# gabrielspmoreira/chameleon_recsys

Measured on AMD Instinct MI355X. Metric: NAR training sessions/sec, higher is better.
Workload: dtype f32

## Files before the change

chameleon_recsys_amd/_lib.py:

```python
import ctypes
import os
from ctypes import c_double, c_float, c_int, c_int32, c_int64, c_long, c_size_t, c_uint32, c_void_p

_HERE = os.path.dirname(os.path.abspath(__file__))
LIB_PATH = os.path.join(_HERE, "libchameleon_nar.so")

P = c_void_p

_SIGNATURES = {
    "cham_neg_sample_workspace_bytes": (c_size_t, [c_int, c_int, c_int]),
    "cham_neg_sample": (c_int, [P, c_int, c_int, P, c_int, c_uint32, c_uint32, c_int, c_int, c_int, c_int, P, P, P, P, P,
                                P, c_size_t, P]),
    "cham_ctx_assemble": (c_int, [P, P, c_int, P, c_int, P, P, P, P, P, P]),
    "cham_set_log_bases": (c_int, [c_float, c_float]),
    "cham_step_ints": (c_int, [P, P, P, P, c_int64, c_int, c_int, P, c_int, P, P, P, P, P, P]),
    "cham_item_dynamic_raw": (c_int, [P, P, c_int, P, P, P, P, P]),
    "cham_norm_stats_from_recent": (c_int, [P, c_int, c_int64, P, P, P, P, P]),
    "cham_norm_stats_from_buffer": (c_int, [P, c_int, c_int64, P, P, P, P, P]),
    "cham_norm_stats_from_rows": (c_int, [P, P, P, c_int, P, P]),
    "cham_row_weights": (c_int, [P, c_int, P, c_size_t, c_int, P, P, P, P]),
    "cham_item_assemble": (c_int, [P, c_int, c_int, c_int, P, c_int, P, c_int, P, P, P, P, c_int, P, P, P, P, P, P]),
    "cham_item_assemble_lds": (c_int, [P, c_int, c_int, c_int, P, c_int, P, c_int, P, P, P, P, c_int, P, c_int, P, c_int, P, P, P, P, P, P]),
    "cham_feature_bwd": (c_int, [P, P, c_int, c_int, P, P, P]),
    "cham_feature_bwd_workspace_bytes": (c_size_t, [c_int]),
# ... 30 lines not shown
    "cham_split2h": (c_int, [P, c_int, c_int, c_int, P, c_int64, c_int, P, c_int64, c_int, P, c_int, P]),
    "cham_gemm_h2": (c_int, [P, c_int64, c_int, P, P, c_int64, c_int, P, c_int, P, c_int, c_int, c_int, c_int, P, c_int, P, c_int, c_int, c_int,
                             P, c_size_t, c_int, P]),
    "cham_h2b_block_elements": (c_int, []),
    "cham_gemm_h2b": (c_int, [P, c_int64, c_int, P, P, c_int64, c_int, P, c_int, P, c_int, c_int, c_int, c_int, P, c_int, P, c_int, c_int, c_int,
                              P, c_size_t, c_int, c_int, c_int, c_int, P]),
    "cham_combine_fwd_h2b": (c_int, [P, P, c_int, c_int, c_int, c_int, P, P, c_int64, P, c_int, P]),
    "cham_dm_mulpred_h2_blk": (c_int, [P, c_int, c_int, P, c_int64, P, P, P, P, c_int, c_int, c_int, P, c_int64, P, P, P, P]),
    "cham_gemm_h2_launch_counts": (None, [P, c_int]),
    "cham_gemm_h2_set_nt_wide": (c_int, [c_int]),
    "cham_combine_fwd_h2": (c_int, [P, P, c_int, c_int, c_int, c_int, P, P, c_int64, P, P]),
    "cham_mulpred_bwd_h2": (c_int, [P, P, P, c_int, c_int, c_int, P, P, c_int64, P, P, P]),
    "cham_dm_mulpred_h2": (c_int, [P, c_int, c_int, P, c_int64, P, P, c_int, c_int, c_int, P, c_int64, P, P, P, P]),
    "cham_dm_mulpred_h2h": (c_int, [P, c_int, c_int, P, c_int64, P, P, P, P, c_int, c_int, c_int, P, c_int64, P, P, P, P]),
    "cham_dm_mulpred_b16": (c_int, [P, c_int, c_int, P, P, P, c_int, c_int, c_int, P, P, P, P]),
    "cham_gemm_b16": (c_int, [P, c_int, c_int, P, c_int, c_int, P, c_int, c_int, c_int, c_int, c_int, P, c_int, P, c_int, c_int, c_int,
                              P, c_size_t, c_int, P]),
    "cham_gemm_b16_set_variant": (None, [c_int]),
    "cham_gemm_b16_launch_counts": (None, [P, c_int]),
    "cham_gemm_set_variant": (None, [c_int]),
    "cham_gemm_launch_counts": (None, [P, c_int]),
    "cham_combine_fwd": (c_int, [P, P, c_int, c_int, c_int, c_int, P, P, c_long, c_long, P]),
    "cham_combine_bwd_workspace_bytes": (c_size_t, [c_int, c_int, c_int, c_int]),
    "cham_combine_bwd": (c_int, [P, c_int, c_int, c_int, c_int, P, P, P, P, c_size_t, P]),
    "cham_combine_bwd_gs": (c_int, [P, c_int, c_int, c_int, c_int, P, P, P, P, c_size_t, P, c_size_t, P]),
    "cham_gemm_h2_groupsum_bytes": (c_size_t, [c_int, c_int, c_int]),
    "cham_gemm_h2_dgrad_gs": (c_int, [P, c_int64, c_int, P, P, c_int64, c_int, P, P, c_int, c_int, c_int, c_int, P, c_int, c_int, c_int, c_int, P,
                                      c_size_t, P]),
    "cham_combine_fwd_b16": (c_int, [P, P, c_int, c_int, c_int, c_int, P, P, P]),
    "cham_combine_bwd_b16": (c_int, [P, P, c_int, c_int, c_int, c_int, P, P, P, P, c_size_t, P]),
# ... 62 lines not shown
def load():
    global _lib
    if _lib is not None:
        return _lib
    if not os.path.exists(LIB_PATH):
        raise ChameleonLibError(
            "HIP extension %s is missing - run `python -c 'import __graft_entry__ as g; g.build()'` "
            "(hipcc --offload-arch=gfx950).  There is no CPU fallback." % LIB_PATH)
    lib = ctypes.CDLL(LIB_PATH)
    for name, (res, args) in _SIGNATURES.items():
        fn = getattr(lib, name)
        fn.restype = res
        fn.argtypes = args
    lib.cham_gemm_h2_set_nt_wide(1 if os.environ.get("CHAM_H2_NT_WIDE", "1") == "1" else 0)
    lib.cham_gemm_b16_dma_set_nt_wide(1 if os.environ.get("CHAM_B16_NT_WIDE", "1") == "1" else 0)
    _lib = lib
    return lib


def check(rc, what):
    if rc != 0:
        raise ChameleonLibError("%s failed with code %d" % (what, rc))


def ptr(t):
    return None if t is None else t.data_ptr()
```

chameleon_recsys_amd/csrc/dm_fused.hip:

```cpp
#include "gemm_shared.h"
#include <type_traits>

#define DMF_NT 2
#define DMF_COLS (32 * DMF_NT)
#define DMF_PLANE (DMF_COLS * 128)
#define DMF_HALF (3 * DMF_PLANE)
#define DMF_RED_OFF (2 * DMF_HALF)
#define DMF_RED_BYTES (8 * 4 * DMF_COLS * 4)

static_assert(DMF_NT == 2, "the epilogue packs exactly two tiles' columns per lane");

struct DmfParams {
    const float* dS1; int lds1;
    const __bf16* W; long long w_ps;
    const float* Z2c; const float* pred;
    __bf16* out; long long out_ps;
    const H2Scale* osc;
    const H2Scale* sa; const H2Scale* sw;
    float* dpred; float* b2part;
    int C, BT, NC, PW;
    int out_blocked;
};

__device__ __forceinline__ void dmf_dma_one(unsigned lds, unsigned voff, const u32x4& r) {
    unsigned keep;
    asm volatile(
        "s_nop 4\n\t"
        "s_mov_b32 %0, m0\n\t"
        "s_mov_b32 m0, %1\n\ts_nop 0\n\tbuffer_load_dwordx4 %2, %3, 0 offen lds\n\t"
        "s_mov_b32 m0, %0"
        : "=&s"(keep) : "s"(lds), "v"(voff), "s"(r) : "memory");
}

template <int MODE>
__global__ __launch_bounds__(512) void k_dm_mulpred_fused(DmfParams p) {
    constexpr bool H2 = MODE == 1 || MODE == 3, B16 = MODE == 2, F16P = MODE == 3;
    constexpr int NPL = B16 ? 1 : (F16P ? 2 : 3);
    extern __shared__ __attribute__((aligned(1024))) unsigned char dmf_smem[];
    const int lane = threadIdx.x & 63, wave = __builtin_amdgcn_readfirstlane(threadIdx.x >> 6);
    const int l31 = lane & 31, hh = lane >> 5;
    const int NC = p.NC, C = p.C;
    const int pos0 = blockIdx.x * p.PW;
    const int npos = min(p.PW, p.BT - pos0);
    const int rows_valid = npos * NC;
    const size_t row0 = (size_t)pos0 * NC;
    const int wr0 = 32 * wave;

    bf16x8 AH[8], AM[(B16 || F16P) ? 1 : 8], AL[B16 ? 1 : 8];
    float ginv_a = 1.f, ginv_w = 1.f;
    if constexpr (B16) {
// ... 20 lines not shown
                                __uint_as_float(x[2 * s + 1].w)};
            if constexpr (F16P) {
                const float sa = p.sa->scale;
#pragma unroll
                for (int e = 0; e < 8; ++e) {
                    _Float16 a, c;
                    split2h(v[e] * sa, a, c);
                    AH[s][e] = __builtin_bit_cast(__bf16, a); AL[s][e] = __builtin_bit_cast(__bf16, c);
                }
            } else {
#pragma unroll
                for (int e = 0; e < 8; ++e) { __bf16 a, b, c; split3(v[e], a, b, c); AH[s][e] = a; AM[s][e] = b; AL[s][e] = c; }
            }
        }
    }
    const __amdgpu_buffer_rsrc_t zw = B16 ?
        __builtin_amdgcn_make_buffer_rsrc(const_cast<__bf16*>(reinterpret_cast<const __bf16*>(p.Z2c) + row0 * (size_t)C), 0,
                                          (unsigned)((size_t)rows_valid * C * 2), 0x00020000) :
        __builtin_amdgcn_make_buffer_rsrc(const_cast<float*>(p.Z2c + row0 * (size_t)C), 0, (unsigned)((size_t)rows_valid * C * 4), 0x00020000);
    __amdgpu_buffer_rsrc_t ow[3];
#pragma unroll
    for (int q = 0; q < 3; ++q)
        ow[q] = __builtin_amdgcn_make_buffer_rsrc(p.out + ((H2 && q == 2) || B16 ? 0 : q) * p.out_ps + row0 * (size_t)C, 0, (unsigned)((size_t)rows_valid * C * 2), 0x00020000);
    const bool oblk = H2 && p.out_blocked != 0;
    const unsigned rin = (unsigned)(row0 & 255), tile_bytes = ((unsigned)C >> 5) * (unsigned)(H2B_BLOCK * 2);
    if (oblk) {
#pragma unroll
        for (int q = 0; q < 2; ++q)
            ow[q] = __builtin_amdgcn_make_buffer_rsrc(p.out + q * p.out_ps + (row0 >> 8) * (size_t)((unsigned)C >> 5) * H2B_BLOCK, 0, 2u * tile_bytes, 0x00020000);
    }
    float osc = 1.f;
    if constexpr (H2) osc = p.osc->scale;
    if constexpr (F16P) { ginv_a = p.sa->inv; ginv_w = p.sw->inv; }

// ... 6 lines not shown
        rw[q].x = (unsigned)a; rw[q].y = (unsigned)(a >> 32) & 0xFFFFu; rw[q].z = (unsigned)((size_t)C * 128 * 2); rw[q].w = 0x00020000u;
    }
    unsigned voff;
    {
        const int slot = 8 * wave + (lane >> 3);
        const int piece = (lane & 7) ^ ((slot >> 1) & 7);
        const int col = DMF_NT * (slot & 31) + (slot >> 5);
        voff = (unsigned)(col * 128 + piece * 8) * 2u;
    }
    auto dma_half = [&](int h) {
        const unsigned base = lds_base + (unsigned)(h & 1) * DMF_HALF + (unsigned)wave * 1024u;
        const unsigned add = (unsigned)(((h >> 1) * DMF_COLS) * 128 + (h & 1) * 64) * 2u;
#pragma unroll
        for (int q = 0; q < NPL; ++q) dmf_dma_one(base + (unsigned)q * DMF_PLANE, voff + add, rw[q]);
    };
    unsigned fo[4];
#pragma unroll
    for (int t = 0; t < 4; ++t) fo[t] = (unsigned)(l31 * 128 + (((2 * t + hh) ^ ((l31 >> 1) & 7)) * 16));

    const int pa = wr0 / NC;
    const int bnd = (pa + 1) * NC - wr0;
    const int ntiles = C / DMF_COLS, nhalf = 2 * ntiles;

    dma_half(0);
    dma_half(1);
    floatx16 acc[DMF_NT];
#pragma unroll
    for (int j = 0; j < DMF_NT; ++j)
#pragma unroll
        for (int e = 0; e < 16; ++e) acc[j][e] = 0.f;
    if constexpr (B16) asm volatile("s_waitcnt vmcnt(1)" ::: "memory");
    else if constexpr (F16P) asm volatile("s_waitcnt vmcnt(2)" ::: "memory");
    else asm volatile("s_waitcnt vmcnt(3)" ::: "memory");
    __builtin_amdgcn_fence(__ATOMIC_RELEASE, "workgroup", "local");
    __builtin_amdgcn_s_barrier();
    __builtin_amdgcn_fence(__ATOMIC_ACQUIRE, "workgroup", "local");

    auto mfma_half = [&](auto PARC) {
        constexpr int PAR = decltype(PARC)::value, s0 = PAR * 4;
        const unsigned char* S = dmf_smem + PAR * DMF_HALF;
        __builtin_amdgcn_sched_barrier(0);
#pragma unroll
        for (int t = 0; t < 4; ++t) {
            bf16x8 bh[DMF_NT], bm[DMF_NT], bl[DMF_NT];
#pragma unroll
            for (int j = 0; j < DMF_NT; ++j) {
                bh[j] = *reinterpret_cast<const bf16x8*>(S + fo[t] + j * 4096);
                if constexpr (F16P) {
// ... 21 lines not shown
#pragma unroll
                for (int j = 0; j < DMF_NT; ++j) acc[j] = __builtin_amdgcn_mfma_f32_32x32x16_bf16(AL[s0 + t], bh[j], acc[j], 0, 0, 0);
#pragma unroll
                for (int j = 0; j < DMF_NT; ++j) acc[j] = __builtin_amdgcn_mfma_f32_32x32x16_bf16(AH[s0 + t], bl[j], acc[j], 0, 0, 0);
#pragma unroll
                for (int j = 0; j < DMF_NT; ++j) acc[j] = __builtin_amdgcn_mfma_f32_32x32x16_bf16(AM[s0 + t], bm[j], acc[j], 0, 0, 0);
#pragma unroll
                for (int j = 0; j < DMF_NT; ++j) acc[j] = __builtin_amdgcn_mfma_f32_32x32x16_bf16(AM[s0 + t], bh[j], acc[j], 0, 0, 0);
#pragma unroll
                for (int j = 0; j < DMF_NT; ++j) acc[j] = __builtin_amdgcn_mfma_f32_32x32x16_bf16(AH[s0 + t], bm[j], acc[j], 0, 0, 0);
#pragma unroll
                for (int j = 0; j < DMF_NT; ++j) acc[j] = __builtin_amdgcn_mfma_f32_32x32x16_bf16(AH[s0 + t], bh[j], acc[j], 0, 0, 0);
            }
        }
    };
    for (int h = 0; h < nhalf; ++h) {
        if (h & 1) mfma_half(std::integral_constant<int, 1>{});
        else mfma_half(std::integral_constant<int, 0>{});
        __builtin_amdgcn_sched_barrier(0);
        asm volatile("s_waitcnt vmcnt(0)" ::: "memory");
        if (h & 1) {
            const int col = (h >> 1) * DMF_COLS + DMF_NT * l31;
            float2 pra = make_float2(0.f, 0.f), prb = pra;
            if (pa < npos) pra = *reinterpret_cast<const float2*>(p.pred + (size_t)(pos0 + pa) * C + col);
            if (pa + 1 < npos) prb = *reinterpret_cast<const float2*>(p.pred + (size_t)(pos0 + pa + 1) * C + col);
            float2 sa = make_float2(0.f, 0.f), sb = sa, ca = sa, cb = sa;
            typedef unsigned int u32x2_t __attribute__((ext_vector_type(2)));
            u32x2_t zz[16];
#pragma unroll
            for (int e = 0; e < 16; ++e) {
                const unsigned r = (unsigned)(wr0 + (e & 3) + 8 * (e >> 2) + 4 * hh);
                if constexpr (B16) {
                    const unsigned u = __builtin_amdgcn_raw_buffer_load_b32(zw, (r * (unsigned)C + (unsigned)col) * 2u, 0, 0);
                    zz[e].x = u << 16; zz[e].y = u & 0xFFFF0000u;
                } else {
                    zz[e] = __builtin_amdgcn_raw_buffer_load_b64(zw, (r * (unsigned)C + (unsigned)col) * 4u, 0, 0);
                }
            }
#pragma unroll
            for (int e = 0; e < 16; ++e) {
                const int rr = (e & 3) + 8 * (e >> 2) + 4 * hh;
                const unsigned r = (unsigned)(wr0 + rr);
                const float2 z = make_float2(__uint_as_float(zz[e].x), __uint_as_float(zz[e].y));
                const bool second = rr >= bnd;
                const float2 pr = second ? prb : pra;
                float2 g = make_float2(acc[0][e], acc[1][e]);
                if constexpr (F16P) { g.x = (g.x * ginv_a) * ginv_w; g.y = (g.y * ginv_a) * ginv_w; }
                if constexpr (B16) { g.x = (float)(__bf16)g.x; g.y = (float)(__bf16)g.y; }
                float2 o;
                o.x = g.x * pr.x * (1.f - z.x * z.x); o.y = g.y * pr.y * (1.f - z.y * z.y);
                if constexpr (B16) {
                    typedef __bf16 bf16x2_t __attribute__((ext_vector_type(2)));
                    bf16x2_t ph; ph[0] = (__bf16)o.x; ph[1] = (__bf16)o.y;
                    __builtin_amdgcn_raw_buffer_store_b32(__builtin_bit_cast(unsigned, ph), ow[0], (r * (unsigned)C + (unsigned)col) * 2u, 0, 0);
                    o.x = (float)ph[0]; o.y = (float)ph[1];
                } else if constexpr (H2) {
                    _Float16 h0, l0, h1, l1;
                    split2h(o.x * osc, h0, l0); split2h(o.y * osc, h1, l1);
                    const unsigned ph = (unsigned)h2_keep_sign(h0, o.x) | ((unsigned)h2_keep_sign(h1, o.y) << 16);
                    const unsigned pl = (unsigned)__builtin_bit_cast(unsigned short, l0) | ((unsigned)__builtin_bit_cast(unsigned short, l1) << 16);
                    unsigned oo = (r * (unsigned)C + (unsigned)col) * 2u;
                    if (oblk) {
                        const unsigned lr = rin + r;
                        oo = (int)r < rows_valid ? (lr >> 8) * tile_bytes + ((unsigned)col >> 5) * (unsigned)(H2B_BLOCK * 2) + (lr & 255u) * 64u + ((unsigned)col & 31u) * 2u
                                                 : 0x80000000u;
                    }
                    __builtin_amdgcn_raw_buffer_store_b32(ph, ow[0], oo, 0, 0);
                    __builtin_amdgcn_raw_buffer_store_b32(pl, ow[1], oo, 0, 0);
                } else {
                    typedef __bf16 bf16x2_t __attribute__((ext_vector_type(2)));
                    bf16x2_t ph, pm, pl;
                    __bf16 a, b, c;
                    split3(o.x, a, b, c); ph[0] = a; pm[0] = b; pl[0] = c;
                    split3(o.y, a, b, c); ph[1] = a; pm[1] = b; pl[1] = c;
                    const unsigned oo = (r * (unsigned)C + (unsigned)col) * 2u;
                    __builtin_amdgcn_raw_buffer_store_b32(__builtin_bit_cast(unsigned, ph), ow[0], oo, 0, 0);
                    __builtin_amdgcn_raw_buffer_store_b32(__builtin_bit_cast(unsigned, pm), ow[1], oo, 0, 0);
                    __builtin_amdgcn_raw_buffer_store_b32(__builtin_bit_cast(unsigned, pl), ow[2], oo, 0, 0);
                }
                const float2 gz = make_float2(g.x * z.x, g.y * z.y);
                sb.x += second ? gz.x : 0.f; sb.y += second ? gz.y : 0.f; cb.x += second ? o.x : 0.f; cb.y += second ? o.y : 0.f;
                sa.x += second ? 0.f : gz.x; sa.y += second ? 0.f : gz.y; ca.x += second ? 0.f : o.x; ca.y += second ? 0.f : o.y;
                acc[0][e] = 0.f; acc[1][e] = 0.f;
            }
            float* red = reinterpret_cast<float*>(dmf_smem + DMF_RED_OFF) + (size_t)wave * (4 * DMF_COLS);
            float2 q[4] = {sa, ca, sb, cb};
#pragma unroll
            for (int i = 0; i < 4; ++i) {
                float2 o;
                o.x = __shfl_xor(q[i].x, 32, 64); o.y = __shfl_xor(q[i].y, 32, 64);
                if (hh == 0) *reinterpret_cast<float2*>(red + i * DMF_COLS + DMF_NT * l31) = make_float2(q[i].x + o.x, q[i].y + o.y);
            }
        }
        __builtin_amdgcn_fence(__ATOMIC_RELEASE, "workgroup", "local");
        __builtin_amdgcn_s_waitcnt(0xc07f);
        __builtin_amdgcn_s_barrier();
        __builtin_amdgcn_fence(__ATOMIC_ACQUIRE, "workgroup", "local");
        if (h & 1) {
            const float* redw = reinterpret_cast<const float*>(dmf_smem + DMF_RED_OFF);
            for (int idx = threadIdx.x; idx < npos * DMF_COLS; idx += 512) {
                const int pl = idx / DMF_COLS, c = idx % DMF_COLS;
                float s = 0.f, cs = 0.f;
                const int w_lo = (pl * NC) >> 5, w_hi = min(7, ((pl + 1) * NC - 1) >> 5);
                for (int w = w_lo; w <= w_hi; ++w) {
                    const int slot = (pl == (32 * w) / NC) ? 0 : 1;
                    s += redw[(size_t)w * (4 * DMF_COLS) + slot * (2 * DMF_COLS) + c];
                    cs += redw[(size_t)w * (4 * DMF_COLS) + slot * (2 * DMF_COLS) + DMF_COLS + c];
                }
                const int colg = (h >> 1) * DMF_COLS + c;
                const float pr = p.pred[(size_t)(pos0 + pl) * C + colg];
                p.dpred[(size_t)(pos0 + pl) * C + colg] = s * (1.f - pr * pr);
                if (p.b2part) p.b2part[(size_t)(pos0 + pl) * C + colg] = cs;
            }
        }
        if (h + 2 < nhalf) dma_half(h + 2);
    }
    asm volatile("s_waitcnt vmcnt(0)" ::: "memory");
}

template <int MODE>
static int dm_mulpred_launch(const float* dS1, int lds1, int K, const void* Wp, long long w_plane_stride, const float* Z2c,
                             const float* pred, int C, int BT, int N, void* dZ2p, long long out_plane_stride, const void* out_scale_rec,
                             float* dpred_pre, float* col_part, void* stream, const void* a_scale_rec = nullptr, const void* w_scale_rec = nullptr,
                             int out_blocked = 0) {
    if (!dS1 || !Wp || !Z2c || !pred || !dZ2p || !dpred_pre || BT < 0 || N < 0 || ((MODE == 1 || MODE == 3) && !out_scale_rec)) return -CHAM_ERR_ARG;
    if (MODE == 3 && (!a_scale_rec || !w_scale_rec || (((uintptr_t)a_scale_rec | (uintptr_t)w_scale_rec) & 3))) return -CHAM_ERR_ARG;
    const int NC = N + 1;
    if (K != 128 || (C % DMF_COLS) || C <= 0 || NC < 32 || NC > 256 || (lds1 & 3) || lds1 < K || (out_plane_stride & 3) || (w_plane_stride & 7))
        return -CHAM_ERR_ARG;
    if (((uintptr_t)dS1 | (uintptr_t)Wp | (uintptr_t)Z2c | (uintptr_t)pred | (uintptr_t)dZ2p) & 15) return -CHAM_ERR_ARG;
    if (out_blocked && ((MODE != 1 && MODE != 3) || (C & 31) || out_plane_stride < (long long)(((size_t)BT * NC + 255) / 256) * (C >> 5) * H2B_BLOCK)) return -CHAM_ERR_ARG;
    if (BT == 0) return CHAM_OK;
    DmfParams p;
    p.out_blocked = out_blocked ? 1 : 0;
    p.dS1 = dS1; p.lds1 = lds1; p.W = reinterpret_cast<const __bf16*>(Wp); p.w_ps = w_plane_stride; p.Z2c = Z2c; p.pred = pred;
    p.out = reinterpret_cast<__bf16*>(dZ2p); p.out_ps = out_plane_stride; p.osc = reinterpret_cast<const H2Scale*>(out_scale_rec);
    p.sa = reinterpret_cast<const H2Scale*>(a_scale_rec); p.sw = reinterpret_cast<const H2Scale*>(w_scale_rec);
    p.dpred = dpred_pre; p.b2part = col_part;
    p.C = C; p.BT = BT; p.NC = NC; p.PW = 256 / NC;
    constexpr int smem = 2 * DMF_HALF + DMF_RED_BYTES;
    auto k = k_dm_mulpred_fused<MODE>;
    CHAM_SET_DYNAMIC_LDS(k, smem);
    hipLaunchKernelGGL(k, dim3((BT + p.PW - 1) / p.PW), dim3(512), smem, (hipStream_t)stream, p);
    CHAM_CHECK_LAUNCH();
    return CHAM_OK;
}

extern "C" int cham_dm_mulpred_p3(const float* dS1, int lds1, int K, const void* Wp, long long w_plane_stride, const float* Z2c,
                                  const float* pred, int C, int BT, int N, void* dZ2p, long long out_plane_stride, float* dpred_pre,
                                  float* col_part, void* stream) {
    return dm_mulpred_launch<0>(dS1, lds1, K, Wp, w_plane_stride, Z2c, pred, C, BT, N, dZ2p, out_plane_stride, nullptr, dpred_pre, col_part, stream);
}

extern "C" int cham_dm_mulpred_h2(const float* dS1, int lds1, int K, const void* Wp, long long w_plane_stride, const float* Z2c,
                                  const float* pred, int C, int BT, int N, void* dZ2p, long long out_plane_stride, const void* out_scale_rec,
                                  float* dpred_pre, float* col_part, void* stream) {
    return dm_mulpred_launch<1>(dS1, lds1, K, Wp, w_plane_stride, Z2c, pred, C, BT, N, dZ2p, out_plane_stride, out_scale_rec, dpred_pre, col_part, stream);
}
// ... 26 lines not shown
```

include/chameleon_nar.h:

```cpp
#ifndef CHAMELEON_NAR_H
#define CHAMELEON_NAR_H
#include <stddef.h>
#include <stdint.h>
#ifdef __cplusplus
extern "C" {
#endif

#define CHAM_ACT_NONE 0
#define CHAM_ACT_LEAKY 1
#define CHAM_ACT_TANH 2

size_t cham_neg_sample_workspace_bytes(int n_aci, int buf_size, int n_from_buffer);
int cham_neg_sample(const int64_t* aci, int Bg, int T1, const int64_t* buffer, int buf_size, uint32_t seed, uint32_t step,
                    int row_begin, int row_count, int N, int n_from_buffer, int64_t* neg_ids, int32_t* neg_slot,
                    int64_t* pool, int32_t* canon, int32_t* meta, void* workspace, size_t workspace_bytes, void* stream);

int cham_ctx_assemble(const int64_t* cat, const float* num, int R, const int64_t* desc, int F, const float* params,
                      const float* gamma, const float* beta, float* xraw, float* xs, void* stream);
int cham_set_log_bases(float elapsed_days_smooth_log_base, float popularity_smooth_log_base);

int cham_step_ints(const int64_t* ic_rows, const int64_t* ln_rows, const int64_t* pool, const int64_t* ets_rows, int64_t max_ts, int BT, int pmax,
                   const int32_t* seq_len_in, int B, const uint8_t* mask_in, int64_t* ids_all, int64_t* ref_ts, int32_t* seq_len, uint8_t* mask,
                   void* stream);

// ... 83 lines not shown
int cham_combine_fwd_h2b(const float* U, const float* V, int C, int BT, int N, int pmax, const int32_t* neg_slot, void* Z1p,
                         long long plane_stride, const void* scale_rec, int blocked, void* stream);
int cham_dm_mulpred_h2_blk(const float* dS1, int lds1, int K, const void* Wp, long long w_plane_stride, const void* ds1_scale_rec,
                           const void* w_scale_rec, const float* Z2c, const float* pred, int C, int BT, int N, void* dZ2p,
                           long long out_plane_stride, const void* out_scale_rec, float* dpred_pre, float* col_part, void* stream);
int cham_combine_fwd_h2(const float* U, const float* V, int C, int BT, int N, int pmax, const int32_t* neg_slot, void* Z1p,
                        long long plane_stride, const void* scale_rec, void* stream);
int cham_mulpred_bwd_h2(const float* dM, const float* Z2c, const float* pred, int C, int BT, int N, float* dpred_pre, void* dZ2p,
                        long long plane_stride, float* col_part, const void* scale_rec, void* stream);
int cham_dm_mulpred_h2(const float* dS1, int lds1, int K, const void* Wp, long long w_plane_stride, const float* Z2c, const float* pred,
                       int C, int BT, int N, void* dZ2p, long long out_plane_stride, const void* out_scale_rec, float* dpred_pre,
                       float* col_part, void* stream);
int cham_dm_mulpred_h2h(const float* dS1, int lds1, int K, const void* Wh, long long w_plane_stride, const void* ds1_scale_rec,
                        const void* w_scale_rec, const float* Z2c, const float* pred, int C, int BT, int N, void* dZ2p,
                        long long out_plane_stride, const void* out_scale_rec, float* dpred_pre, float* col_part, void* stream);
int cham_dm_mulpred_b16(const void* dS1, int lds1, int K, const void* Ws1b, const void* Z2c, const float* pred, int C, int BT, int N, void* dZ2c,
                        float* dpred_pre, float* col_part, void* stream);

int cham_combine_fwd_p3(const float* U, const float* V, int C, int BT, int N, int pmax, const int32_t* neg_slot, void* Z1p,
                        long long plane_stride, void* stream);
int cham_mulpred_bwd_p3(const float* dM, const float* Z2c, const float* pred, int C, int BT, int N, float* dpred_pre, void* dZ2p,
                        long long plane_stride, float* col_part, void* stream);

int cham_dm_mulpred_p3(const float* dS1, int lds1, int K, const void* Wp, long long w_plane_stride, const float* Z2c, const float* pred,
                       int C, int BT, int N, void* dZ2p, long long out_plane_stride, float* dpred_pre, float* col_part, void* stream);

int cham_gemm_b16(const void* A, int lda, int transA, const void* B, int ldb, int transB, void* C, int ldc, int out_f32, int M,
                  int N, int K, const float* bias, int act, const void* dref, int ldr, int dact, int accumulate, float* workspace,
                  size_t workspace_bytes, int splits_hint, void* stream);
void cham_gemm_b16_set_variant(int variant);
// ... 129 lines not shown
```

Baseline: 34710.

## Stage Z2c tiles into LDS via async DMA in fused dM-mulpred kernel

The fused dM/mulpred backward kernel now prefetches each wave's Z2c tile into LDS with buffer-load-to-LDS DMA, overlapped with the MFMA half-tiles, instead of issuing per-element global loads in the epilogue. The loop is restructured per column tile: the next B-operand DMA is issued earlier, and pred values are loaded via buffer loads that overlap the second MFMA half. The dpred reduction is simplified to one position per wave. Old behaviour is kept as a 'direct' kernel behind an env toggle, and the FMA contraction pattern for 1-z^2 is pinned per mode to keep numerics stable. The cost is extra LDS per block and more intricate waitcnt/barrier sequencing.

```diff
diff --git a/chameleon_recsys_amd/_lib.py b/chameleon_recsys_amd/_lib.py
--- a/chameleon_recsys_amd/_lib.py
+++ b/chameleon_recsys_amd/_lib.py
@@ -68,6 +68,7 @@
     "cham_dm_mulpred_h2": (c_int, [P, c_int, c_int, P, c_int64, P, P, c_int, c_int, c_int, P, c_int64, P, P, P, P]),
     "cham_dm_mulpred_h2h": (c_int, [P, c_int, c_int, P, c_int64, P, P, P, P, c_int, c_int, c_int, P, c_int64, P, P, P, P]),
     "cham_dm_mulpred_b16": (c_int, [P, c_int, c_int, P, P, P, c_int, c_int, c_int, P, P, P, P]),
+    "cham_dm_mulpred_set_staged": (c_int, [c_int]),
     "cham_gemm_b16": (c_int, [P, c_int, c_int, P, c_int, c_int, P, c_int, c_int, c_int, c_int, c_int, P, c_int, P, c_int, c_int, c_int,
                               P, c_size_t, c_int, P]),
     "cham_gemm_b16_set_variant": (None, [c_int]),
@@ -160,6 +161,7 @@
         fn.argtypes = args
     lib.cham_gemm_h2_set_nt_wide(1 if os.environ.get("CHAM_H2_NT_WIDE", "1") == "1" else 0)
     lib.cham_gemm_b16_dma_set_nt_wide(1 if os.environ.get("CHAM_B16_NT_WIDE", "1") == "1" else 0)
+    lib.cham_dm_mulpred_set_staged(1 if os.environ.get("CHAM_DM_STAGED", "1") == "1" else 0)
     _lib = lib
     return lib
 
diff --git a/chameleon_recsys_amd/csrc/dm_fused.hip b/chameleon_recsys_amd/csrc/dm_fused.hip
--- a/chameleon_recsys_amd/csrc/dm_fused.hip
+++ b/chameleon_recsys_amd/csrc/dm_fused.hip
@@ -7,6 +7,8 @@
 #define DMF_HALF (3 * DMF_PLANE)
 #define DMF_RED_OFF (2 * DMF_HALF)
 #define DMF_RED_BYTES (8 * 4 * DMF_COLS * 4)
+#define DMF_ZST_OFF (DMF_RED_OFF + DMF_RED_BYTES)
+#define DMF_ZST_WAVE(es) (32 * DMF_COLS * (es))
 
 static_assert(DMF_NT == 2, "the epilogue packs exactly two tiles' columns per lane");
 
@@ -33,7 +35,20 @@
 }
 
 template <int MODE>
+__global__ __launch_bounds__(512) void k_dm_mulpred_direct(DmfParams p) {
+#include "dm_fused_direct_body.h"
+}
+
+
+__host__ __device__ constexpr unsigned dmf_usq_fused(int mode) { return mode == 3 ? 0xFFFFu : (mode == 1 ? 0xFF00u : 0u); }
+__host__ __device__ constexpr bool dmf_staged_mode(int mode) { return mode != 0; }
+__device__ __forceinline__ float dmf_mul_rounded(float a, float b) {
+#pragma clang fp contract(off)
+    return a * b;
+}
+template <int MODE>
 __global__ __launch_bounds__(512) void k_dm_mulpred_fused(DmfParams p) {
+    static_assert(dmf_staged_mode(MODE), "MODE 0 has no staged form: the specialisation below");
     constexpr bool H2 = MODE == 1 || MODE == 3, B16 = MODE == 2, F16P = MODE == 3;
     constexpr int NPL = B16 ? 1 : (F16P ? 2 : 3);
     extern __shared__ __attribute__((aligned(1024))) unsigned char dmf_smem[];
@@ -84,10 +99,15 @@
             }
         }
     }
-    const __amdgpu_buffer_rsrc_t zw = B16 ?
-        __builtin_amdgcn_make_buffer_rsrc(const_cast<__bf16*>(reinterpret_cast<const __bf16*>(p.Z2c) + row0 * (size_t)C), 0,
-                                          (unsigned)((size_t)rows_valid * C * 2), 0x00020000) :
-        __builtin_amdgcn_make_buffer_rsrc(const_cast<float*>(p.Z2c + row0 * (size_t)C), 0, (unsigned)((size_t)rows_valid * C * 4), 0x00020000);
+    constexpr unsigned ZES = B16 ? 2u : 4u, ZROWB = DMF_COLS * ZES, ZLPR = ZROWB / 16u, ZRPQ = 64u / ZLPR, ZNQ = 32u / ZRPQ;
+    u32x4 rz;
+    {
+        const unsigned long long a = (unsigned long long)(reinterpret_cast<const unsigned char*>(p.Z2c) + row0 * (size_t)C * ZES);
+        rz.x = (unsigned)a; rz.y = (unsigned)(a >> 32) & 0xFFFFu; rz.z = (unsigned)((size_t)rows_valid * C * ZES); rz.w = 0x00020000u;
+    }
+    const unsigned zvoff = (((unsigned)wr0 + (unsigned)lane / ZLPR) * (unsigned)C) * ZES + ((unsigned)lane % ZLPR) * 16u;
+    const __amdgpu_buffer_rsrc_t pw = __builtin_amdgcn_make_buffer_rsrc(const_cast<float*>(p.pred + (size_t)pos0 * C), 0,
+                                                                        (unsigned)((size_t)npos * C * 4), 0x00020000);
     __amdgpu_buffer_rsrc_t ow[3];
 #pragma unroll
     for (int q = 0; q < 3; ++q)
@@ -124,24 +144,29 @@
 #pragma unroll
         for (int q = 0; q < NPL; ++q) dmf_dma_one(base + (unsigned)q * DMF_PLANE, voff + add, rw[q]);
     };
+    auto zdma = [&](int t) {
+        const unsigned base = lds_base + DMF_ZST_OFF + (unsigned)wave * DMF_ZST_WAVE(ZES);
+        const unsigned add = (unsigned)t * ZROWB;
+#pragma unroll
+        for (unsigned i = 0; i < ZNQ; ++i) dmf_dma_one(base + i * 1024u, zvoff + add + i * ZRPQ * (unsigned)C * ZES, rz);
+    };
     unsigned fo[4];
 #pragma unroll
     for (int t = 0; t < 4; ++t) fo[t] = (unsigned)(l31 * 128 + (((2 * t + hh) ^ ((l31 >> 1) & 7)) * 16));
 
     const int pa = wr0 / NC;
     const int bnd = (pa + 1) * NC - wr0;
-    const int ntiles = C / DMF_COLS, nhalf = 2 * ntiles;
+    const int ntiles = C / DMF_COLS;
 
     dma_half(0);
     dma_half(1);
+    zdma(0);
     floatx16 acc[DMF_NT];
 #pragma unroll
     for (int j = 0; j < DMF_NT; ++j)
 #pragma unroll
         for (int e = 0; e < 16; ++e) acc[j][e] = 0.f;
-    if constexpr (B16) asm volatile("s_waitcnt vmcnt(1)" ::: "memory");
-    else if constexpr (F16P) asm volatile("s_waitcnt vmcnt(2)" ::: "memory");
-    else asm volatile("s_waitcnt vmcnt(3)" ::: "memory");
+    asm volatile("s_waitcnt vmcnt(%0)" :: "n"(NPL + (int)ZNQ) : "memory");
     __builtin_amdgcn_fence(__ATOMIC_RELEASE, "workgroup", "local");
     __builtin_amdgcn_s_barrier();
     __builtin_amdgcn_fence(__ATOMIC_ACQUIRE, "workgroup", "local");
@@ -193,41 +218,64 @@
             }
         }
     };
-    for (int h = 0; h < nhalf; ++h) {
-        if (h & 1) mfma_half(std::integral_constant<int, 1>{});
-        else mfma_half(std::integral_constant<int, 0>{});
+    auto sync = [&]() {
+        __builtin_amdgcn_fence(__ATOMIC_RELEASE, "workgroup", "local");
+        __builtin_amdgcn_s_waitcnt(0xc07f);
+        __builtin_amdgcn_s_barrier();
+        __builtin_amdgcn_fence(__ATOMIC_ACQUIRE, "workgroup", "local");
+    };
+    for (int t = 0; t < ntiles; ++t) {
+        const bool more = t + 1 < ntiles;
+        const unsigned c0 = (unsigned)t * DMF_COLS;
+        mfma_half(std::integral_constant<int, 0>{});
         __builtin_amdgcn_sched_barrier(0);
         asm volatile("s_waitcnt vmcnt(0)" ::: "memory");
-        if (h & 1) {
-            const int col = (h >> 1) * DMF_COLS + DMF_NT * l31;
-            float2 pra = make_float2(0.f, 0.f), prb = pra;
-            if (pa < npos) pra = *reinterpret_cast<const float2*>(p.pred + (size_t)(pos0 + pa) * C + col);
-            if (pa + 1 < npos) prb = *reinterpret_cast<const float2*>(p.pred + (size_t)(pos0 + pa + 1) * C + col);
+        sync();
+        if (more) dma_half(2 * t + 2);
+        typedef unsigned int u32x2_t __attribute__((ext_vector_type(2)));
+        u32x2_t ua = __builtin_amdgcn_raw_buffer_load_b64(pw, ((unsigned)pa * (unsigned)C + c0 + DMF_NT * (unsigned)l31) * 4u, 0, 0);
+        u32x2_t ub = __builtin_amdgcn_raw_buffer_load_b64(pw, ((unsigned)(pa + 1) * (unsigned)C + c0 + DMF_NT * (unsigned)l31) * 4u, 0, 0);
+        unsigned uc = __builtin_amdgcn_raw_buffer_load_b32(pw, ((unsigned)wave * (unsigned)C + c0 + (unsigned)lane) * 4u, 0, 0);
+        mfma_half(std::integral_constant<int, 1>{});
+        __builtin_amdgcn_sched_barrier(0);
+        asm volatile("s_waitcnt vmcnt(0)" ::: "memory");
+        asm volatile("" : "+v"(ua.x), "+v"(ua.y), "+v"(ub.x), "+v"(ub.y), "+v"(uc));
+        const float2 pra = make_float2(__uint_as_float(ua.x), __uint_as_float(ua.y)), prb = make_float2(__uint_as_float(ub.x), __uint_as_float(ub.y));
+        {
+            const int col = (int)c0 + DMF_NT * l31;
             float2 sa = make_float2(0.f, 0.f), sb = sa, ca = sa, cb = sa;
-            typedef unsigned int u32x2_t __attribute__((ext_vector_type(2)));
             u32x2_t zz[16];
+            const unsigned char* zs = dmf_smem + DMF_ZST_OFF + (unsigned)wave * DMF_ZST_WAVE(ZES) + (unsigned)hh * (4u * ZROWB) + (unsigned)l31 * (2u * ZES);
 #pragma unroll
             for (int e = 0; e < 16; ++e) {
-                const unsigned r = (unsigned)(wr0 + (e & 3) + 8 * (e >> 2) + 4 * hh);
-                if constexpr (B16) {
-                    const unsigned u = __builtin_amdgcn_raw_buffer_load_b32(zw, (r * (unsigned)C + (unsigned)col) * 2u, 0, 0);
-                    zz[e].x = u << 16; zz[e].y = u & 0xFFFF0000u;
-                } else {
-                    zz[e] = __builtin_amdgcn_raw_buffer_load_b64(zw, (r * (unsigned)C + (unsigned)col) * 4u, 0, 0);
-                }
-            }
+                const unsigned ro = (unsigned)((e & 3) + 8 * (e >> 2)) * ZROWB;
+                if constexpr (B16) zz[e].x = *reinterpret_cast<const unsigned*>(zs + ro);
+                else zz[e] = *reinterpret_cast<const u32x2_t*>(zs + ro);
+            }
+            asm volatile("s_waitcnt lgkmcnt(0)" ::: "memory");
+            if (more) zdma(t + 1);
 #pragma unroll
             for (int e = 0; e < 16; ++e) {
                 const int rr = (e & 3) + 8 * (e >> 2) + 4 * hh;
                 const unsigned r = (unsigned)(wr0 + rr);
-                const float2 z = make_float2(__uint_as_float(zz[e].x), __uint_as_float(zz[e].y));
+                const bool valid = (int)r < rows_valid;
+                float2 z;
+                if constexpr (B16) {
+                    const unsigned u = valid ? zz[e].x : 0u;
+                    z = make_float2(__uint_as_float(u << 16), __uint_as_float(u & 0xFFFF0000u));
+                } else {
+                    z = make_float2(__uint_as_float(valid ? zz[e].x : 0u), __uint_as_float(valid ? zz[e].y : 0u));
+                }
                 const bool second = rr >= bnd;
                 const float2 pr = second ? prb : pra;
                 float2 g = make_float2(acc[0][e], acc[1][e]);
                 if constexpr (F16P) { g.x = (g.x * ginv_a) * ginv_w; g.y = (g.y * ginv_a) * ginv_w; }
                 if constexpr (B16) { g.x = (float)(__bf16)g.x; g.y = (float)(__bf16)g.y; }
+                float2 u;
+                if ((dmf_usq_fused(MODE) >> e) & 1u) { u.x = __builtin_fmaf(-z.x, z.x, 1.f); u.y = __builtin_fmaf(-z.y, z.y, 1.f); }
+                else { u.x = 1.f - dmf_mul_rounded(z.x, z.x); u.y = 1.f - dmf_mul_rounded(z.y, z.y); }
                 float2 o;
-                o.x = g.x * pr.x * (1.f - z.x * z.x); o.y = g.y * pr.y * (1.f - z.y * z.y);
+                o.x = g.x * pr.x * u.x; o.y = g.y * pr.y * u.y;
                 if constexpr (B16) {
                     typedef __bf16 bf16x2_t __attribute__((ext_vector_type(2)));
                     bf16x2_t ph; ph[0] = (__bf16)o.x; ph[1] = (__bf16)o.y;
@@ -241,8 +289,8 @@
                     unsigned oo = (r * (unsigned)C + (unsigned)col) * 2u;
                     if (oblk) {
                         const unsigned lr = rin + r;
-                        oo = (int)r < rows_valid ? (lr >> 8) * tile_bytes + ((unsigned)col >> 5) * (unsigned)(H2B_BLOCK * 2) + (lr & 255u) * 64u + ((unsigned)col & 31u) * 2u
-                                                 : 0x80000000u;
+                        oo = valid ? (lr >> 8) * tile_bytes + ((unsigned)col >> 5) * (unsigned)(H2B_BLOCK * 2) + (lr & 255u) * 64u + ((unsigned)col & 31u) * 2u
+                                   : 0x80000000u;
                     }
                     __builtin_amdgcn_raw_buffer_store_b32(ph, ow[0], oo, 0, 0);
                     __builtin_amdgcn_raw_buffer_store_b32(pl, ow[1], oo, 0, 0);
@@ -271,31 +319,35 @@
                 if (hh == 0) *reinterpret_cast<float2*>(red + i * DMF_COLS + DMF_NT * l31) = make_float2(q[i].x + o.x, q[i].y + o.y);
             }
         }
-        __builtin_amdgcn_fence(__ATOMIC_RELEASE, "workgroup", "local");
-        __builtin_amdgcn_s_waitcnt(0xc07f);
-        __builtin_amdgcn_s_barrier();
-        __builtin_amdgcn_fence(__ATOMIC_ACQUIRE, "workgroup", "local");
-        if (h & 1) {
+        sync();
+        if ((int)threadIdx.x < npos * DMF_COLS) {
             const float* redw = reinterpret_cast<const float*>(dmf_smem + DMF_RED_OFF);
-            for (int idx = threadIdx.x; idx < npos * DMF_COLS; idx += 512) {
-                const int pl = idx / DMF_COLS, c = idx % DMF_COLS;
-                float s = 0.f, cs = 0.f;
-                const int w_lo = (pl * NC) >> 5, w_hi = min(7, ((pl + 1) * NC - 1) >> 5);
-                for (int w = w_lo; w <= w_hi; ++w) {
-                    const int slot = (pl == (32 * w) / NC) ? 0 : 1;
-                    s += redw[(size_t)w * (4 * DMF_COLS) + slot * (2 * DMF_COLS) + c];
-                    cs += redw[(size_t)w * (4 * DMF_COLS) + slot * (2 * DMF_COLS) + DMF_COLS + c];
-                }
-                const int colg = (h >> 1) * DMF_COLS + c;
-                const float pr = p.pred[(size_t)(pos0 + pl) * C + colg];
-                p.dpred[(size_t)(pos0 + pl) * C + colg] = s * (1.f - pr * pr);
-                if (p.b2part) p.b2part[(size_t)(pos0 + pl) * C + colg] = cs;
-            }
+            const int pl = wave, c = lane;
+            float s = 0.f, cs = 0.f;
+            const int w_lo = (pl * NC) >> 5, w_hi = min(7, ((pl + 1) * NC - 1) >> 5);
+            for (int w = w_lo; w <= w_hi; ++w) {
+                const int slot = (pl == (32 * w) / NC) ? 0 : 1;
+                s += redw[(size_t)w * (4 * DMF_COLS) + slot * (2 * DMF_COLS) + c];
+                cs += redw[(size_t)w * (4 * DMF_COLS) + slot * (2 * DMF_COLS) + DMF_COLS + c];
+            }
+            const int colg = (int)c0 + c;
+            const float pr = __uint_as_float(uc);
+            p.dpred[(size_t)(pos0 + pl) * C + colg] = s * __builtin_fmaf(-pr, pr, 1.f);
+            if (p.b2part) p.b2part[(size_t)(pos0 + pl) * C + colg] = cs;
         }
-        if (h + 2 < nhalf) dma_half(h + 2);
+        if (more) dma_half(2 * t + 3);
     }
     asm volatile("s_waitcnt vmcnt(0)" ::: "memory");
 }
+
+template <>
+__global__ __launch_bounds__(512) void k_dm_mulpred_fused<0>(DmfParams p) {
+    constexpr int MODE = 0;
+#include "dm_fused_direct_body.h"
+}
+
+static int g_dm_staged = 1;
+extern "C" int cham_dm_mulpred_set_staged(int on) { const int was = g_dm_staged; g_dm_staged = on ? 1 : 0; return was; }
 
 template <int MODE>
 static int dm_mulpred_launch(const float* dS1, int lds1, int K, const void* Wp, long long w_plane_stride, const float* Z2c,
@@ -317,10 +369,22 @@
     p.sa = reinterpret_cast<const H2Scale*>(a_scale_rec); p.sw = reinterpret_cast<const H2Scale*>(w_scale_rec);
     p.dpred = dpred_pre; p.b2part = col_part;
     p.C = C; p.BT = BT; p.NC = NC; p.PW = 256 / NC;
-    constexpr int smem = 2 * DMF_HALF + DMF_RED_BYTES;
-    auto k = k_dm_mulpred_fused<MODE>;
-    CHAM_SET_DYNAMIC_LDS(k, smem);
-    hipLaunchKernelGGL(k, dim3((BT + p.PW - 1) / p.PW), dim3(512), smem, (hipStream_t)stream, p);
+    const dim3 grid((BT + p.PW - 1) / p.PW);
+    constexpr int smem_direct = 2 * DMF_HALF + DMF_RED_BYTES;
+    if constexpr (!dmf_staged_mode(MODE)) {
+        auto k = k_dm_mulpred_fused<MODE>;
+        CHAM_SET_DYNAMIC_LDS(k, smem_direct);
+        hipLaunchKernelGGL(k, grid, dim3(512), smem_direct, (hipStream_t)stream, p);
+    } else if (g_dm_staged) {
+        constexpr int smem = DMF_ZST_OFF + 8 * DMF_ZST_WAVE(MODE == 2 ? 2 : 4);
+        auto k = k_dm_mulpred_fused<MODE>;
+        CHAM_SET_DYNAMIC_LDS(k, smem);
+        hipLaunchKernelGGL(k, grid, dim3(512), smem, (hipStream_t)stream, p);
+    } else {
+        auto k = k_dm_mulpred_direct<MODE>;
+        CHAM_SET_DYNAMIC_LDS(k, smem_direct);
+        hipLaunchKernelGGL(k, grid, dim3(512), smem_direct, (hipStream_t)stream, p);
+    }
     CHAM_CHECK_LAUNCH();
     return CHAM_OK;
 }
diff --git a/chameleon_recsys_amd/csrc/dm_fused_direct_body.h b/chameleon_recsys_amd/csrc/dm_fused_direct_body.h
--- /dev/null
+++ b/chameleon_recsys_amd/csrc/dm_fused_direct_body.h
@@ -0,0 +1,261 @@
+    constexpr bool H2 = MODE == 1 || MODE == 3, B16 = MODE == 2, F16P = MODE == 3;
+    constexpr int NPL = B16 ? 1 : (F16P ? 2 : 3);
+    extern __shared__ __attribute__((aligned(1024))) unsigned char dmf_smem[];
+    const int lane = threadIdx.x & 63, wave = __builtin_amdgcn_readfirstlane(threadIdx.x >> 6);
+    const int l31 = lane & 31, hh = lane >> 5;
+    const int NC = p.NC, C = p.C;
+    const int pos0 = blockIdx.x * p.PW;
+    const int npos = min(p.PW, p.BT - pos0);
+    const int rows_valid = npos * NC;
+    const size_t row0 = (size_t)pos0 * NC;
+    const int wr0 = 32 * wave;
+
+    bf16x8 AH[8], AM[(B16 || F16P) ? 1 : 8], AL[B16 ? 1 : 8];
+    float ginv_a = 1.f, ginv_w = 1.f;
+    if constexpr (B16) {
+        const __bf16* a16 = reinterpret_cast<const __bf16*>(p.dS1);
+        const __amdgpu_buffer_rsrc_t aw = __builtin_amdgcn_make_buffer_rsrc(const_cast<__bf16*>(a16 + row0 * (size_t)p.lds1), 0,
+                                                                            (unsigned)((size_t)rows_valid * p.lds1 * 2), 0x00020000);
+        const unsigned ao = ((unsigned)(wr0 + l31) * (unsigned)p.lds1 + 8u * hh) * 2u;
+#pragma unroll
+        for (int s = 0; s < 8; ++s) AH[s] = __builtin_bit_cast(bf16x8, __builtin_amdgcn_raw_buffer_load_b128(aw, ao + 32u * s, 0, 0));
+    } else {
+        const __amdgpu_buffer_rsrc_t aw = __builtin_amdgcn_make_buffer_rsrc(const_cast<float*>(p.dS1 + row0 * (size_t)p.lds1), 0,
+                                                                            (unsigned)((size_t)rows_valid * p.lds1 * 4), 0x00020000);
+        const unsigned ao = ((unsigned)(wr0 + l31) * (unsigned)p.lds1 + 8u * hh) * 4u;
+        u32x4 x[16];
+#pragma unroll
+        for (int s = 0; s < 8; ++s) {
+            x[2 * s] = __builtin_amdgcn_raw_buffer_load_b128(aw, ao + 64u * s, 0, 0);
+            x[2 * s + 1] = __builtin_amdgcn_raw_buffer_load_b128(aw, ao + 64u * s + 16u, 0, 0);
+        }
+#pragma unroll
+        for (int s = 0; s < 8; ++s) {
+            const float v[8] = {__uint_as_float(x[2 * s].x), __uint_as_float(x[2 * s].y), __uint_as_float(x[2 * s].z), __uint_as_float(x[2 * s].w),
+                                __uint_as_float(x[2 * s + 1].x), __uint_as_float(x[2 * s + 1].y), __uint_as_float(x[2 * s + 1].z),
+                                __uint_as_float(x[2 * s + 1].w)};
+            if constexpr (F16P) {
+                const float sa = p.sa->scale;
+#pragma unroll
+                for (int e = 0; e < 8; ++e) {
+                    _Float16 a, c;
+                    split2h(v[e] * sa, a, c);
+                    AH[s][e] = __builtin_bit_cast(__bf16, a); AL[s][e] = __builtin_bit_cast(__bf16, c);
+                }
+            } else {
+#pragma unroll
+                for (int e = 0; e < 8; ++e) { __bf16 a, b, c; split3(v[e], a, b, c); AH[s][e] = a; AM[s][e] = b; AL[s][e] = c; }
+            }
+        }
+    }
+    const __amdgpu_buffer_rsrc_t zw = B16 ?
+        __builtin_amdgcn_make_buffer_rsrc(const_cast<__bf16*>(reinterpret_cast<const __bf16*>(p.Z2c) + row0 * (size_t)C), 0,
+                                          (unsigned)((size_t)rows_valid * C * 2), 0x00020000) :
+        __builtin_amdgcn_make_buffer_rsrc(const_cast<float*>(p.Z2c + row0 * (size_t)C), 0, (unsigned)((size_t)rows_valid * C * 4), 0x00020000);
+    __amdgpu_buffer_rsrc_t ow[3];
+#pragma unroll
+    for (int q = 0; q < 3; ++q)
+        ow[q] = __builtin_amdgcn_make_buffer_rsrc(p.out + ((H2 && q == 2) || B16 ? 0 : q) * p.out_ps + row0 * (size_t)C, 0, (unsigned)((size_t)rows_valid * C * 2), 0x00020000);
+    const bool oblk = H2 && p.out_blocked != 0;
+    const unsigned rin = (unsigned)(row0 & 255), tile_bytes = ((unsigned)C >> 5) * (unsigned)(H2B_BLOCK * 2);
+    if (oblk) {
+#pragma unroll
+        for (int q = 0; q < 2; ++q)
+            ow[q] = __builtin_amdgcn_make_buffer_rsrc(p.out + q * p.out_ps + (row0 >> 8) * (size_t)((unsigned)C >> 5) * H2B_BLOCK, 0, 2u * tile_bytes, 0x00020000);
+    }
+    float osc = 1.f;
+    if constexpr (H2) osc = p.osc->scale;
+    if constexpr (F16P) { ginv_a = p.sa->inv; ginv_w = p.sw->inv; }
+
+    typedef __attribute__((address_space(3))) unsigned char lds_u8;
+    const unsigned lds_base = (unsigned)(unsigned long long)(lds_u8*)dmf_smem;
+    u32x4 rw[3];
+#pragma unroll
+    for (int q = 0; q < 3; ++q) {
+        const unsigned long long a = (unsigned long long)(p.W + q * p.w_ps);
+        rw[q].x = (unsigned)a; rw[q].y = (unsigned)(a >> 32) & 0xFFFFu; rw[q].z = (unsigned)((size_t)C * 128 * 2); rw[q].w = 0x00020000u;
+    }
+    unsigned voff;
+    {
+        const int slot = 8 * wave + (lane >> 3);
+        const int piece = (lane & 7) ^ ((slot >> 1) & 7);
+        const int col = DMF_NT * (slot & 31) + (slot >> 5);
+        voff = (unsigned)(col * 128 + piece * 8) * 2u;
+    }
+    auto dma_half = [&](int h) {
+        const unsigned base = lds_base + (unsigned)(h & 1) * DMF_HALF + (unsigned)wave * 1024u;
+        const unsigned add = (unsigned)(((h >> 1) * DMF_COLS) * 128 + (h & 1) * 64) * 2u;
+#pragma unroll
+        for (int q = 0; q < NPL; ++q) dmf_dma_one(base + (unsigned)q * DMF_PLANE, voff + add, rw[q]);
+    };
+    unsigned fo[4];
+#pragma unroll
+    for (int t = 0; t < 4; ++t) fo[t] = (unsigned)(l31 * 128 + (((2 * t + hh) ^ ((l31 >> 1) & 7)) * 16));
+
+    const int pa = wr0 / NC;
+    const int bnd = (pa + 1) * NC - wr0;
+    const int ntiles = C / DMF_COLS, nhalf = 2 * ntiles;
+
+    dma_half(0);
+    dma_half(1);
+    floatx16 acc[DMF_NT];
+#pragma unroll
+    for (int j = 0; j < DMF_NT; ++j)
+#pragma unroll
+        for (int e = 0; e < 16; ++e) acc[j][e] = 0.f;
+    if constexpr (B16) asm volatile("s_waitcnt vmcnt(1)" ::: "memory");
+    else if constexpr (F16P) asm volatile("s_waitcnt vmcnt(2)" ::: "memory");
+    else asm volatile("s_waitcnt vmcnt(3)" ::: "memory");
+    __builtin_amdgcn_fence(__ATOMIC_RELEASE, "workgroup", "local");
+    __builtin_amdgcn_s_barrier();
+    __builtin_amdgcn_fence(__ATOMIC_ACQUIRE, "workgroup", "local");
+
+    auto mfma_half = [&](auto PARC) {
+        constexpr int PAR = decltype(PARC)::value, s0 = PAR * 4;
+        const unsigned char* S = dmf_smem + PAR * DMF_HALF;
+        __builtin_amdgcn_sched_barrier(0);
+#pragma unroll
+        for (int t = 0; t < 4; ++t) {
+            bf16x8 bh[DMF_NT], bm[DMF_NT], bl[DMF_NT];
+#pragma unroll
+            for (int j = 0; j < DMF_NT; ++j) {
+                bh[j] = *reinterpret_cast<const bf16x8*>(S + fo[t] + j * 4096);
+                if constexpr (F16P) {
+                    bl[j] = *reinterpret_cast<const bf16x8*>(S + DMF_PLANE + fo[t] + j * 4096);
+                } else if constexpr (!B16) {
+                    bm[j] = *reinterpret_cast<const bf16x8*>(S + DMF_PLANE + fo[t] + j * 4096);
+                    bl[j] = *reinterpret_cast<const bf16x8*>(S + 2 * DMF_PLANE + fo[t] + j * 4096);
+                }
+            }
+            if constexpr (F16P) {
+                typedef _Float16 dmf_half8 __attribute__((ext_vector_type(8)));
+#pragma unroll
+                for (int j = 0; j < DMF_NT; ++j)
+                    acc[j] = __builtin_amdgcn_mfma_f32_32x32x16_f16(__builtin_bit_cast(dmf_half8, AL[s0 + t]), __builtin_bit_cast(dmf_half8, bh[j]), acc[j], 0, 0, 0);
+#pragma unroll
+                for (int j = 0; j < DMF_NT; ++j)
+                    acc[j] = __builtin_amdgcn_mfma_f32_32x32x16_f16(__builtin_bit_cast(dmf_half8, AH[s0 + t]), __builtin_bit_cast(dmf_half8, bl[j]), acc[j], 0, 0, 0);
+#pragma unroll
+                for (int j = 0; j < DMF_NT; ++j)
+                    acc[j] = __builtin_amdgcn_mfma_f32_32x32x16_f16(__builtin_bit_cast(dmf_half8, AH[s0 + t]), __builtin_bit_cast(dmf_half8, bh[j]), acc[j], 0, 0, 0);
+            } else if constexpr (B16) {
+#pragma unroll
+                for (int j = 0; j < DMF_NT; ++j) acc[j] = __builtin_amdgcn_mfma_f32_32x32x16_bf16(AH[s0 + t], bh[j], acc[j], 0, 0, 0);
+            } else {
+#pragma unroll
+                for (int j = 0; j < DMF_NT; ++j) acc[j] = __builtin_amdgcn_mfma_f32_32x32x16_bf16(AL[s0 + t], bh[j], acc[j], 0, 0, 0);
+#pragma unroll
+                for (int j = 0; j < DMF_NT; ++j) acc[j] = __builtin_amdgcn_mfma_f32_32x32x16_bf16(AH[s0 + t], bl[j], acc[j], 0, 0, 0);
+#pragma unroll
+                for (int j = 0; j < DMF_NT; ++j) acc[j] = __builtin_amdgcn_mfma_f32_32x32x16_bf16(AM[s0 + t], bm[j], acc[j], 0, 0, 0);
+#pragma unroll
+                for (int j = 0; j < DMF_NT; ++j) acc[j] = __builtin_amdgcn_mfma_f32_32x32x16_bf16(AM[s0 + t], bh[j], acc[j], 0, 0, 0);
+#pragma unroll
+                for (int j = 0; j < DMF_NT; ++j) acc[j] = __builtin_amdgcn_mfma_f32_32x32x16_bf16(AH[s0 + t], bm[j], acc[j], 0, 0, 0);
+#pragma unroll
+                for (int j = 0; j < DMF_NT; ++j) acc[j] = __builtin_amdgcn_mfma_f32_32x32x16_bf16(AH[s0 + t], bh[j], acc[j], 0, 0, 0);
+            }
+        }
+    };
+    for (int h = 0; h < nhalf; ++h) {
+        if (h & 1) mfma_half(std::integral_constant<int, 1>{});
+        else mfma_half(std::integral_constant<int, 0>{});
+        __builtin_amdgcn_sched_barrier(0);
+        asm volatile("s_waitcnt vmcnt(0)" ::: "memory");
+        if (h & 1) {
+            const int col = (h >> 1) * DMF_COLS + DMF_NT * l31;
+            float2 pra = make_float2(0.f, 0.f), prb = pra;
+            if (pa < npos) pra = *reinterpret_cast<const float2*>(p.pred + (size_t)(pos0 + pa) * C + col);
+            if (pa + 1 < npos) prb = *reinterpret_cast<const float2*>(p.pred + (size_t)(pos0 + pa + 1) * C + col);
+            float2 sa = make_float2(0.f, 0.f), sb = sa, ca = sa, cb = sa;
+            typedef unsigned int u32x2_t __attribute__((ext_vector_type(2)));
+            u32x2_t zz[16];
+#pragma unroll
+            for (int e = 0; e < 16; ++e) {
+                const unsigned r = (unsigned)(wr0 + (e & 3) + 8 * (e >> 2) + 4 * hh);
+                if constexpr (B16) {
+                    const unsigned u = __builtin_amdgcn_raw_buffer_load_b32(zw, (r * (unsigned)C + (unsigned)col) * 2u, 0, 0);
+                    zz[e].x = u << 16; zz[e].y = u & 0xFFFF0000u;
+                } else {
+                    zz[e] = __builtin_amdgcn_raw_buffer_load_b64(zw, (r * (unsigned)C + (unsigned)col) * 4u, 0, 0);
+                }
+            }
+#pragma unroll
+            for (int e = 0; e < 16; ++e) {
+                const int rr = (e & 3) + 8 * (e >> 2) + 4 * hh;
+                const unsigned r = (unsigned)(wr0 + rr);
+                const float2 z = make_float2(__uint_as_float(zz[e].x), __uint_as_float(zz[e].y));
+                const bool second = rr >= bnd;
+                const float2 pr = second ? prb : pra;
+                float2 g = make_float2(acc[0][e], acc[1][e]);
+                if constexpr (F16P) { g.x = (g.x * ginv_a) * ginv_w; g.y = (g.y * ginv_a) * ginv_w; }
+                if constexpr (B16) { g.x = (float)(__bf16)g.x; g.y = (float)(__bf16)g.y; }
+                float2 o;
+                o.x = g.x * pr.x * (1.f - z.x * z.x); o.y = g.y * pr.y * (1.f - z.y * z.y);
+                if constexpr (B16) {
+                    typedef __bf16 bf16x2_t __attribute__((ext_vector_type(2)));
+                    bf16x2_t ph; ph[0] = (__bf16)o.x; ph[1] = (__bf16)o.y;
+                    __builtin_amdgcn_raw_buffer_store_b32(__builtin_bit_cast(unsigned, ph), ow[0], (r * (unsigned)C + (unsigned)col) * 2u, 0, 0);
+                    o.x = (float)ph[0]; o.y = (float)ph[1];
+                } else if constexpr (H2) {
+                    _Float16 h0, l0, h1, l1;
+                    split2h(o.x * osc, h0, l0); split2h(o.y * osc, h1, l1);
+                    const unsigned ph = (unsigned)h2_keep_sign(h0, o.x) | ((unsigned)h2_keep_sign(h1, o.y) << 16);
+                    const unsigned pl = (unsigned)__builtin_bit_cast(unsigned short, l0) | ((unsigned)__builtin_bit_cast(unsigned short, l1) << 16);
+                    unsigned oo = (r * (unsigned)C + (unsigned)col) * 2u;
+                    if (oblk) {
+                        const unsigned lr = rin + r;
+                        oo = (int)r < rows_valid ? (lr >> 8) * tile_bytes + ((unsigned)col >> 5) * (unsigned)(H2B_BLOCK * 2) + (lr & 255u) * 64u + ((unsigned)col & 31u) * 2u
+                                                 : 0x80000000u;
+                    }
+                    __builtin_amdgcn_raw_buffer_store_b32(ph, ow[0], oo, 0, 0);
+                    __builtin_amdgcn_raw_buffer_store_b32(pl, ow[1], oo, 0, 0);
+                } else {
+                    typedef __bf16 bf16x2_t __attribute__((ext_vector_type(2)));
+                    bf16x2_t ph, pm, pl;
+                    __bf16 a, b, c;
+                    split3(o.x, a, b, c); ph[0] = a; pm[0] = b; pl[0] = c;
+                    split3(o.y, a, b, c); ph[1] = a; pm[1] = b; pl[1] = c;
+                    const unsigned oo = (r * (unsigned)C + (unsigned)col) * 2u;
+                    __builtin_amdgcn_raw_buffer_store_b32(__builtin_bit_cast(unsigned, ph), ow[0], oo, 0, 0);
+                    __builtin_amdgcn_raw_buffer_store_b32(__builtin_bit_cast(unsigned, pm), ow[1], oo, 0, 0);
+                    __builtin_amdgcn_raw_buffer_store_b32(__builtin_bit_cast(unsigned, pl), ow[2], oo, 0, 0);
+                }
+                const float2 gz = make_float2(g.x * z.x, g.y * z.y);
+                sb.x += second ? gz.x : 0.f; sb.y += second ? gz.y : 0.f; cb.x += second ? o.x : 0.f; cb.y += second ? o.y : 0.f;
+                sa.x += second ? 0.f : gz.x; sa.y += second ? 0.f : gz.y; ca.x += second ? 0.f : o.x; ca.y += second ? 0.f : o.y;
+                acc[0][e] = 0.f; acc[1][e] = 0.f;
+            }
+            float* red = reinterpret_cast<float*>(dmf_smem + DMF_RED_OFF) + (size_t)wave * (4 * DMF_COLS);
+            float2 q[4] = {sa, ca, sb, cb};
+#pragma unroll
+            for (int i = 0; i < 4; ++i) {
+                float2 o;
+                o.x = __shfl_xor(q[i].x, 32, 64); o.y = __shfl_xor(q[i].y, 32, 64);
+                if (hh == 0) *reinterpret_cast<float2*>(red + i * DMF_COLS + DMF_NT * l31) = make_float2(q[i].x + o.x, q[i].y + o.y);
+            }
+        }
+        __builtin_amdgcn_fence(__ATOMIC_RELEASE, "workgroup", "local");
+        __builtin_amdgcn_s_waitcnt(0xc07f);
+        __builtin_amdgcn_s_barrier();
+        __builtin_amdgcn_fence(__ATOMIC_ACQUIRE, "workgroup", "local");
+        if (h & 1) {
+            const float* redw = reinterpret_cast<const float*>(dmf_smem + DMF_RED_OFF);
+            for (int idx = threadIdx.x; idx < npos * DMF_COLS; idx += 512) {
+                const int pl = idx / DMF_COLS, c = idx % DMF_COLS;
+                float s = 0.f, cs = 0.f;
+                const int w_lo = (pl * NC) >> 5, w_hi = min(7, ((pl + 1) * NC - 1) >> 5);
+                for (int w = w_lo; w <= w_hi; ++w) {
+                    const int slot = (pl == (32 * w) / NC) ? 0 : 1;
+                    s += redw[(size_t)w * (4 * DMF_COLS) + slot * (2 * DMF_COLS) + c];
+                    cs += redw[(size_t)w * (4 * DMF_COLS) + slot * (2 * DMF_COLS) + DMF_COLS + c];
+                }
+                const int colg = (h >> 1) * DMF_COLS + c;
+                const float pr = p.pred[(size_t)(pos0 + pl) * C + colg];
+                p.dpred[(size_t)(pos0 + pl) * C + colg] = s * (1.f - pr * pr);
+                if (p.b2part) p.b2part[(size_t)(pos0 + pl) * C + colg] = cs;
+            }
+        }
+        if (h + 2 < nhalf) dma_half(h + 2);
+    }
+    asm volatile("s_waitcnt vmcnt(0)" ::: "memory");
diff --git a/include/chameleon_nar.h b/include/chameleon_nar.h
--- a/include/chameleon_nar.h
+++ b/include/chameleon_nar.h
@@ -121,6 +121,7 @@
 int cham_dm_mulpred_h2h(const float* dS1, int lds1, int K, const void* Wh, long long w_plane_stride, const void* ds1_scale_rec,
                         const void* w_scale_rec, const float* Z2c, const float* pred, int C, int BT, int N, void* dZ2p,
                         long long out_plane_stride, const void* out_scale_rec, float* dpred_pre, float* col_part, void* stream);
+int cham_dm_mulpred_set_staged(int on);
 int cham_dm_mulpred_b16(const void* dS1, int lds1, int K, const void* Ws1b, const void* Z2c, const float* pred, int C, int BT, int N, void* dZ2c,
                         float* dpred_pre, float* col_part, void* stream);
 
```

Result: no change. 34780, median of 2 (+0.2%).
